# DonghuiZhuo/kube-batch-1

Measured on AMD Instinct MI355X. Metric: pod placements/sec + p50 session latency, 100k nodes × 1M pods, higher is better.
Workload: dtype int64

## Files before the change

kube-batch-1_amd/csrc/engine/engine_placer.h:

```cpp
#pragma once
#include <hip/hip_runtime.h>

#define KBHIP_STAMPS_OFF
#include "../kbhip_batch.h"
#include "../kbhip_engine.h"
#include "engine_dev.h"

namespace kbhip {

static_assert(sizeof(Row) == 4 * (kPkFlags - kPkRow), "the package carries a Row as 28 32-bit words");
static_assert(kEngDescClass + sizeof(TaskClass) / 4 <= kEngDescWords, "a descriptor carries its class");

template <typename ET>
__device__ __forceinline__ Row eng_row_after(const TaskClass& c, const PlaceDec<ET>& D, const Row& base) {
    const int cc = D.cc > 0 ? D.cc : 0;
    const int na = cc < D.ap_l ? cc : D.ap_l;
    return apply_commits(base, c, na, cc - na);
}
template <typename ET>
__device__ __forceinline__ void eng_fit_vals(const Conf& cf, const NodeCols& nc, const DevTables& t,
                                             const TaskClass& c, const PopArgs& a, const PlaceDec<ET>& D,
                                             const Row& base, const int32_t* fit_in, uint32_t fit_raw, uint64_t* g0,
                                             uint64_t* g1) {
    uint32_t fb_base = 0, fb_post = 0;
// ... 127 lines not shown

__device__ __forceinline__ void eng_host_out(const EngArgs& A, EngPlacerLds& L, uint32_t p, uint32_t slot) {
    const int lane = threadIdx.x & 63;
    while (__hip_atomic_load(&L.gran_seq, __ATOMIC_RELAXED, __HIP_MEMORY_SCOPE_WORKGROUP) != (int)p) {
        if (!__hip_atomic_load(&L.ok, __ATOMIC_RELAXED, __HIP_MEMORY_SCOPE_WORKGROUP)) return;
        __builtin_amdgcn_s_sleep(1);
    }
    PopOut* out = (PopOut*)((char*)A.out + (size_t)slot * sizeof(PopOut));
    const uint64_t g = L.gran[lane];
    if (lane < 2 && L.gfit[lane])
        __hip_atomic_store(&out->fit[lane], L.gfit[lane], __ATOMIC_RELAXED, __HIP_MEMORY_SCOPE_SYSTEM);
    if (g) __hip_atomic_store(&out->g[lane], g, __ATOMIC_RELAXED, __HIP_MEMORY_SCOPE_SYSTEM);
    ETL(A, p, 8);
}

__device__ __forceinline__ void eng_drop_stale(EngPlacerLds& L, const PopArgs& a, uint32_t q) {
    const int lane = threadIdx.x & 63;
    EngRowCache& rc = L.rc;
    const int r1 = (int)((q + 3) % 4);
    const int stage = kEngStage + kEngPkgN * (int)(q % 2);
    L.s64[lane] = 0;
    const uint32_t k0 = L.pkey[q % 2][lane], k1 = L.pkey[q % 2][64 + lane];
    auto kept = [&](uint32_t k) {
        if (!k) return false;
        const int sl = rc_find(&rc, key_node(k, a));
        return !(sl >= 64 * r1 && sl < 64 * r1 + 64);
    };
    const bool c0 = kept(k0), c1 = kept(k1);
    const uint64_t m0 = __ballot(c0), m1 = __ballot(c1);
    const int q0 = __builtin_amdgcn_mbcnt_hi((uint32_t)(m0 >> 32), __builtin_amdgcn_mbcnt_lo((uint32_t)m0, 0));
    const int q1 = __popcll(m0) +
                   __builtin_amdgcn_mbcnt_hi((uint32_t)(m1 >> 32), __builtin_amdgcn_mbcnt_lo((uint32_t)m1, 0));
    __builtin_amdgcn_s_waitcnt(0xc07f);
    __builtin_amdgcn_wave_barrier();
    if (c0) L.s64[q0] = k0;
    if (c1 && q1 < 64) L.s64[q1] = k1;
    if (c0) rc_insert(&rc, key_node(k0, a), stage + lane);
    if (c1 && q1 < 64) rc_insert(&rc, key_node(k1, a), stage + 64 + lane);
}

struct FrontKey {
    uint32_t e, fb, kind;
    int32_t na, s1p;
};
__device__ __forceinline__ FrontKey front_key(const Conf& cf, const NodeCols& nc, const DevTables& t,
                                              const TaskClass& c, const PopArgs& a, int node, const Row& r,
                                              uint8_t fl) {
    FrontKey k{0u, 0u, 0u, 0, INT32_MIN};
    const uint64_t pw[4] = {0, 0, 0, 0};
    int32_t sc;
    bool passed;
    const bool st = static_pred_f(cf, c, t, nc, node, fl);
    k.na = (st && cf.score_mult) ? na_weight(c, t, nc, node) : 0;
    const uint64_t k0 = dyn_key(cf, c, t, nc, r, pw, node, st, k.na, &sc, &passed);
    k.e = sweep_key<uint32_t>(k0, a);
    k.fb = fit_bits(c, r, passed);
    k.kind = k0 ? key_kind(k0) : 0;
    if (__ballot(k.kind == 2) != 0 && k.kind == 2) {
        const uint64_t k1 = dyn_key(cf, c, t, nc, apply_commits(r, c, 0, 1), pw, node, true, k.na, &sc, &passed);
        k.s1p = k1 ? key_score(k1) : INT32_MIN;
    }
    return k;
}
__device__ __forceinline__ int32_t front_s1a(const Conf& cf, const NodeCols& nc, const DevTables& t,
                                             const TaskClass& c, int node, const Row& r) {
    const uint64_t pw[4] = {0, 0, 0, 0};
    int32_t sc;
    bool passed;
    const int32_t na = cf.score_mult ? na_weight(c, t, nc, node) : 0;
    const uint64_t k1 = dyn_key(cf, c, t, nc, apply_commits(r, c, 1, 0), pw, node, true, na, &sc, &passed);
    return k1 ? key_score(k1) : INT32_MIN;
}
__device__ __forceinline__ bool front_wait(const EngPlacerLds& L, const int* seq, int want) {
    while (__hip_atomic_load(seq, __ATOMIC_RELAXED, __HIP_MEMORY_SCOPE_WORKGROUP) != want) {
        if (!__hip_atomic_load(&L.ok, __ATOMIC_RELAXED, __HIP_MEMORY_SCOPE_WORKGROUP)) return false;
        __builtin_amdgcn_s_sleep(1);
    }
    return true;
}

template <bool LIST>
__device__ __forceinline__ void eng_front_eval(const Conf& cf, const NodeCols& nc, const DevTables& t,
                                               const EngArgs& A, EngPlacerLds& L, uint32_t q, uint32_t dw, int set,
                                               int role) {
    const int lane = eng_lane();
    uint32_t w[8];
#pragma unroll
    for (int i = 0; i < 8; ++i) w[i] = (uint32_t)__builtin_amdgcn_readlane((int)dw, i);
    const EngDesc d = eng_decode(w);
    const PopArgs a = eng_args(d);
    const TaskClass c = eng_class_x(dw);
    const int ring = (int)((q + 3 - set) % 4);
    const int sl = 64 * ring + lane;
    if (!LIST && set == 0) {
        if (!front_wait(L, &L.rows_seq, (int)(q - 1))) return;
        const int node = L.xn[ring][lane];
        if (role == 0) {
            ETL(A, q - 1, 32);
            FrontKey k{0u, 0u, 0u, 0, INT32_MIN};
            if (node >= 0) k = front_key(cf, nc, t, c, a, node, L.rc.row[sl], L.flags[sl]);
            ETL(A, q - 1, 33);
            L.fe[0][lane] = k.e;
            L.ffb[0][lane] = (uint8_t)k.fb;
            L.fkind[0][lane] = (uint8_t)k.kind;
            L.fna[0][lane] = k.na;
            if (k.kind == 2) L.fs1p[0][lane] = k.s1p;
            ETL(A, q - 1, 34);
            L.e[0][lane] = wave_sort_desc(node >= 0 ? k.e : 0u);
            L.fbp[0][lane] = node >= 0 ? (uint8_t)k.fb : (uint8_t)0;
            __builtin_amdgcn_s_waitcnt(0xc07f);
            if (lane == 0) __hip_atomic_store(&L.sort_seq[0], (int)q, __ATOMIC_RELAXED, __HIP_MEMORY_SCOPE_WORKGROUP);
            ETL(A, q - 1, 35);
// ... 473 lines not shown
```

kube-batch-1_amd/csrc/kbhip_batch.h:

```cpp
#pragma once
#include <hip/hip_runtime.h>

#include "kbhip_eval.h"
#include "kbhip_internal.h"

namespace kbhip {

#if defined(KBHIP_STAMPS) && !defined(KBHIP_STAMPS_OFF)
static __device__ uint64_t* g_stamps;
#define STAMP(slot)                                                       \
    do {                                                                  \
        if (threadIdx.x == 0) g_stamps[(slot)] = __builtin_amdgcn_s_memrealtime(); \
    } while (0)
#else
#define STAMP(slot) do {} while (0)
#endif

#ifdef KBHIP_TIMELINE
constexpr int kTlSlots = 32768, kTlEvents = 32;
constexpr int kTlbSamples = 512, kTlbBlocks = 256;
static __constant__ uint64_t* g_tl;
#define TL(seq, ev)                                                                             \
    do {                                                                                        \
        if (g_tl) g_tl[((seq) % kTlSlots) * kTlEvents + (ev)] = __builtin_amdgcn_s_memrealtime(); \
// ... 717 lines not shown
        } else {
            const int32_t s0 = key_score(K), sm = key_score(Km);
            const int32_t rm = s1d < s0 ? s1d : s0;
            reach = rm > sm || (rm == sm && n < key_idx(Km));
        }
    }
    uint64_t alive = __ballot(reach);
    const int ap_own = K && key_kind(K) == 2 ? 0 : 64;
    if (Km && !alive && !every_member) {
        const bool inm = lane < m;
        const ET L = inm ? depth_entry<ET>(key_score(K), n, 0, a) : (ET)0;
        return tail(true, L, inm, lane, inm ? key_kind(K) : 0, ap_own);
    }
    q_cnt[lane] = 0;
    q_apos[lane] = ap_own;
    q_rm[lane] = K ? key_score(K) : 0;
    q_dl[lane] = 0;
    q_kind[0][lane] = K ? (uint8_t)key_kind(K) : (uint8_t)0;
    for (int h = lane; h < kHash; h += 64) q_hkey[h] = -1;
    __builtin_amdgcn_s_waitcnt(0xc07f);
    __builtin_amdgcn_wave_barrier();
    if (n >= 0) {
        int h = hash_slot(n);
        while (atomicCAS(&q_hkey[h], -1, n) != -1) h = (h + 1) & (kHash - 1);
        q_hlane[h] = lane;
    }
    ET L = K ? depth_entry<ET>(key_score(K), n, 0, a) : (ET)0;
    while (alive) {
        const int k = __popcll(alive);
        const int lk = k <= 1 ? 0 : k <= 2 ? 1 : k <= 4 ? 2 : k <= 8 ? 3 : k <= 16 ? 4 : k <= 32 ? 5 : 6;
        const int Dd = 64 >> lk;
        if ((alive >> lane) & 1)
            q_rl[__builtin_amdgcn_mbcnt_hi((uint32_t)(alive >> 32), __builtin_amdgcn_mbcnt_lo((uint32_t)alive, 0))] = lane;
        q_alive[lane] = 0;
        __builtin_amdgcn_s_waitcnt(0xc07f);
        __builtin_amdgcn_wave_barrier();
        const int seg = lane >> (6 - lk), off = lane & (Dd - 1);
        int j = seg < k ? q_rl[seg] : -1;
        const int dl = j >= 0 ? q_dl[j] : 0;
        const int d = dl + 1 + off;
        const int lastoff = (Dd < 63 - dl ? Dd : 63 - dl) - 1;
        if (off > lastoff) j = -1;
        Row bj{};
        int32_t naj = 0, rm0 = 0;
        int nj = -1, apj = 64;
        if (j >= 0) {
            const int sl = rc_slots[j];
            nj = key_idx(K0[j]);
            bj = rc->row[sl];
            naj = rc->na[sl];
            rm0 = q_rm[j];
            apj = q_apos[j];
        }
        auto eval_at = [&](int dd, int ap, int32_t* sc) -> int {
            const int na = dd < ap ? dd : ap;
            const Row r = apply_commits(bj, c, na, dd - na);
            int32_t s = 0;
            bool passed;
            const uint64_t kk = dyn_key(cf, c, t, nc, r, pw, nj, true, naj, &s, &passed);
            *sc = kk ? key_score(kk) : 0;
            return kk ? key_kind(kk) : 0;
        };
        int32_t sc = 0;
        int kd = j >= 0 ? eval_at(d, apj, &sc) : 0;
        int ap = (j >= 0 && kd == 2) ? d : 64;
        for (int o = 1; o < Dd; o <<= 1) {
            const int x = __shfl_xor(ap, o, 64);
            ap = x < ap ? x : ap;
        }
        ap = apj < ap ? apj : ap;
        const bool redo = j >= 0 && apj == 64 && d > ap;
        if (__ballot(redo) != 0 && redo) kd = eval_at(d, ap, &sc);
        bool ok = j >= 0 && kd != 0;
        int32_t rm = sc;
        for (int o = 1; o < Dd; o <<= 1) {
            const int32_t x = __shfl_up(rm, o, 64);
            const int y = __shfl_up((int)ok, o, 64);
            if (off >= o) {
                rm = x < rm ? x : rm;
                ok = ok && y;
            }
        }
        rm = rm0 < rm ? rm0 : rm;
        const ET e = ok ? depth_entry<ET>(rm, nj, d, a) : (ET)0;
        if (j >= 0) q_kind[d][j] = (uint8_t)kd;
        L = wave_merge_desc(L, wave_sort_desc(e));
        const ET T = readlane_t(L, m - 1);
        if (j >= 0 && off == lastoff) {
            q_rm[j] = rm;
            q_dl[j] = d;
            q_apos[j] = ap;
            q_alive[j] = (e != 0 && e >= T && d < 63) ? 1 : 0;
        }
        __builtin_amdgcn_s_waitcnt(0xc07f);
        __builtin_amdgcn_wave_barrier();
        alive = __ballot(q_alive[lane] != 0);
    }
    const bool inm = lane < m && L != 0;
    int lf = 0;
    if (inm) {
        const int ni = entry_node(L, a);
        int h = hash_slot(ni);
        while (q_hkey[h] != ni) h = (h + 1) & (kHash - 1);
        lf = q_hlane[h];
    }
    const int kind = inm ? q_kind[entry_depth(L)][lf] : 0;
    return tail(false, L, inm, lf, kind, q_apos[lane]);
}

template <typename ET>
__device__ __forceinline__ void place_fit_vals(const Conf& cf, const NodeCols& nc, const DevTables& t,
                                               const TaskClass& c, const PopArgs& a, const PlaceDec<ET>& D,
// ... 395 lines not shown
```

kube-batch-1_amd/csrc/kbhip_eval.h:

```cpp
#pragma once
#include <hip/hip_runtime.h>

#include <cmath>

#include "kbhip_internal.h"

#define KBHIP_HD __host__ __device__ __forceinline__

namespace kbhip {

struct Row {
    int64_t idle_cpu, idle_mem, idle_gpu, rel_cpu, rel_mem, rel_gpu, bf_cpu, bf_mem, bf_gpu;
    int64_t acpu, amem, nzc, nzm;
    int32_t pods, maxtasks;
};

struct ShardCand {
    uint64_t key;
    int32_t node;
    int32_t na;
    Row row;
    uint64_t pw[4];
};
struct ShardMsg {
// ... 52 lines not shown
        }
        case OP_EXISTS: return v >= 0;
        case OP_DNE: return v < 0;
        case OP_GT: return v >= 0 && t.valok[v] && t.valint[v] > r.rhs;
        case OP_LT: return v >= 0 && t.valok[v] && t.valint[v] < r.rhs;
    }
    return false;
}

KBHIP_HD bool term_match(const DevTables& t, const NodeCols& nc, const Term& tm, int n) {
    bool ok = true;
    for (int i = 0; i < tm.req_n; ++i) ok = ok && req_match(t, nc, t.reqs[tm.req_off + i], n);
    return ok;
}

KBHIP_HD bool static_pred_f(const Conf& cf, const TaskClass& c, const DevTables& t, const NodeCols& nc, int n,
                            uint8_t flags) {
    if (!cf.pred_on) return true;
    if (c.pred_err) return false;
    if (flags & 1) return false;
    for (int w = 0; w < nc.taint_words; ++w)
        if (nc.taints[(int64_t)w * nc.npad + n] & ~t.masks[c.tol_off + w]) return false;
    if (c.nsel_term >= 0 && !term_match(t, nc, t.terms[c.nsel_term], n)) return false;
    if (c.req_term_n >= 0) {
        bool any = false;
        for (int i = 0; i < c.req_term_n; ++i) any = any || term_match(t, nc, t.terms[c.req_term_off + i], n);
        if (!any) return false;
    }
    return true;
}
KBHIP_HD bool static_pred(const Conf& cf, const TaskClass& c, const DevTables& t, const NodeCols& nc, int n) {
    return static_pred_f(cf, c, t, nc, n, cf.pred_on ? nc.flags[n] : (uint8_t)0);
}

KBHIP_HD int32_t na_weight(const TaskClass& c, const DevTables& t, const NodeCols& nc, int n) {
    int32_t na = 0;
    for (int i = 0; i < c.pref_term_n; ++i) {
        const Term& tm = t.terms[c.pref_term_off + i];
        if (term_match(t, nc, tm, n)) na += tm.weight;
    }
    return na;
}

KBHIP_HD int64_t lr_score_f(int64_t req, int64_t cap, double f) {
    if (cap == 0 || req > cap) return 0;
    const int64_t num = (cap - req) * 10;
    int64_t q = (int64_t)(10.0 - 10.0 * f);
    q = q < 0 ? 0 : (q > 10 ? 10 : q);
    if (q * cap > num) --q;
    if ((q + 1) * cap <= num) ++q;
    return q;
}

KBHIP_HD int32_t node_score(const Conf& cf, const TaskClass& c, const Row& r, int32_t na, int32_t ipa) {
    if (!cf.score_mult) return 0;
    const int64_t rc = c.nz_cpu + r.nzc, rm = c.nz_mem + r.nzm;
    const double cpuF = r.acpu == 0 ? 1.0 : (double)rc / (double)r.acpu;
    const double memF = r.amem == 0 ? 1.0 : (double)rm / (double)r.amem;
    const int64_t lr = (lr_score_f(rc, r.acpu, cpuF) + lr_score_f(rm, r.amem, memF)) / 2;
    int64_t bra = 0;
    if (!(cpuF >= 1.0 || memF >= 1.0)) {
        const double d = fabs(cpuF - memF);
        const double one_minus = 1.0 - d;
        bra = (int64_t)(one_minus * 10.0);
    }
    return ((int32_t)lr * cf.w_lr + (int32_t)bra * cf.w_bra + na * cf.w_na + ipa * cf.w_pa) * cf.score_mult;
}

KBHIP_HD uint64_t dyn_key(const Conf& cf, const TaskClass& c, const DevTables& t,
                                            const NodeCols& nc, const Row& r, const uint64_t* portw,
                                            int n, bool stat_ok, int32_t na, int32_t* score_out, bool* passed,
                                            int32_t ipa = 0) {
    bool ok = stat_ok;
    if (cf.pred_on) {
        if (r.maxtasks <= r.pods) ok = false;
        if (c.has_ports)
            for (int w = 0; w < 4; ++w) if (w < port_win(c, nc))
                if (portw[w] & t.masks[c.pconf_off + w]) ok = false;
    }
    if (ok && c.score_err) ok = false;
    *passed = ok;
    if (!ok) return 0;
    const int32_t s = node_score(cf, c, r, na, ipa);
    *score_out = s;
    const bool fit_acc = c.ireq_cpu - (r.idle_cpu + r.bf_cpu) < kMinCPU &&
                         c.ireq_mem - (r.idle_mem + r.bf_mem) < kMinMem &&
                         c.ireq_gpu - (r.idle_gpu + r.bf_gpu) < kMinGPU;
    const bool fit_rel = c.ireq_cpu - r.rel_cpu < kMinCPU && c.ireq_mem - r.rel_mem < kMinMem &&
                         c.ireq_gpu - r.rel_gpu < kMinGPU;
    if (!fit_acc && !fit_rel) return 0;
    return pack_key(s, n + nc.base, fit_acc ? 0 : 1);
}

KBHIP_HD uint32_t fit_bits(const TaskClass& c, const Row& r, bool passed) {
    if (!passed) return 0;
    const int64_t ic = r.idle_cpu + r.bf_cpu, im = r.idle_mem + r.bf_mem, ig = r.idle_gpu + r.bf_gpu;
    const int64_t dc = c.req_cpu > 0 ? ic - (c.req_cpu + kMinCPU) : ic;
    const int64_t dm = c.req_mem > 0 ? im - (c.req_mem + kMinMem) : im;
    const int64_t dg = c.req_gpu > 0 ? ig - (c.req_gpu + kMinGPU) : ig;
    return 1u | (dc < 0 ? 2u : 0u) | (dm < 0 ? 4u : 0u) | (dg < 0 ? 8u : 0u);
}

KBHIP_HD uint64_t eval_node(const Conf& cf, const TaskClass& c, const DevTables& t,
                                              const NodeCols& nc, int n, int32_t* score_out, bool* passed,
                                              uint32_t* fit = nullptr) {
    const uint8_t fl = nc.flags[n];
    const Row r = load_row(nc, n);
    uint64_t pw[4] = {0, 0, 0, 0};
    if (c.has_ports)
        for (int w = 0; w < 4; ++w) if (w < port_win(c, nc)) pw[w] = nc.ports[port_at(c, nc, w, n)];
    const bool st = static_pred_f(cf, c, t, nc, n, fl);
    const int32_t na = (st && cf.score_mult) ? na_weight(c, t, nc, n) : 0;
    const uint64_t k = dyn_key(cf, c, t, nc, r, pw, n, st, na, score_out, passed);
    if (fit) *fit = fit_bits(c, r, *passed);
    return k;
}

KBHIP_HD uint64_t eval_node_walk(const Conf& cf, const TaskClass& c, const DevTables& t,
                                 const NodeCols& nc, int n, uint32_t* fit) {
    const Row r = load_row(nc, n);
    uint64_t pw[4] = {0, 0, 0, 0};
    if (c.has_ports)
        for (int w = 0; w < 4; ++w) if (w < port_win(c, nc)) pw[w] = nc.ports[port_at(c, nc, w, n)];
    const bool st = static_pred(cf, c, t, nc, n);
    const int32_t na = (st && cf.score_mult) ? na_weight(c, t, nc, n) : 0;
    int32_t s = 0;
    bool passed = false;
    uint64_t k = dyn_key(cf, c, t, nc, r, pw, n, st, na, &s, &passed);
    if (!k && passed && (r.bf_cpu | r.bf_mem | r.bf_gpu)) k = pack_key(s, n + nc.base, 0);
    *fit = fit_bits(c, r, passed);
    return k;
}

KBHIP_HD int32_t dom_g(const NodeCols& nc, int space, int g) {
    return nc.dom[(int64_t)space * nc.dom_stride + g];
}
// ... 128 lines not shown
```

kube-batch-1_amd/csrc/kbhip_types.h:

```cpp
#pragma once
#include <stdint.h>

namespace kbhip {

constexpr int kBlock = 256;
constexpr int kTopK = 64;
constexpr int kMaxChunk = 64;
constexpr int64_t kMinCPU = 10, kMinGPU = 10, kMinMem = 10LL * 1024 * 1024;

struct NodeCols {
    int64_t *idle_cpu, *idle_mem, *idle_gpu;
    int64_t *rel_cpu, *rel_mem, *rel_gpu;
    int64_t *bf_cpu, *bf_mem, *bf_gpu;
    int64_t *acpu, *amem;
    int64_t *nzc, *nzm;
    int32_t *pods, *maxtasks;
    uint8_t *flags;
    uint32_t *visits;
    int32_t *labels;
    uint64_t *taints;
    uint64_t *ports;
    int32_t *dom;
    int32_t n, npad, n_keys, taint_words, port_words;
    int32_t base;
    int32_t dom_stride;
};

enum : int32_t { OP_IN = 0, OP_NOTIN = 1, OP_EXISTS = 2, OP_DNE = 3, OP_GT = 4, OP_LT = 5,
                 OP_NAME_IN = 6, OP_NAME_NOTIN = 7, OP_FALSE = 8 };
struct Req {
    int32_t key;
    int32_t op;
    int32_t nvals;
    int32_t val_off;
    int64_t rhs;
};
struct Term {
    int32_t req_off, req_n;
    int32_t weight;
    int32_t pad;
};

struct TaskClass {
    int64_t ireq_cpu, ireq_mem, ireq_gpu;
    int64_t req_cpu, req_mem, req_gpu;
    int64_t nz_cpu, nz_mem;
    int32_t backfill;
    int32_t nsel_term;
    int32_t req_term_off, req_term_n;
    int32_t pref_term_off, pref_term_n;
    int32_t tol_off;
    int32_t pconf_off;
    int32_t pown_off;
    int32_t has_ports;
    int32_t pred_err;
    int32_t score_err;
    int32_t aff;
    int32_t ea_off, ea_n;
    int32_t pa_space, pa_cnt, pa_total, pa_self;
    int32_t paa_space, paa_cnt;
    int32_t ipa_off, ipa_n;
    int32_t upd_off, upd_n;
    int32_t pw_lo;
    int32_t dd_space;
    int32_t dd_ndom;
};
constexpr int kDedupMax = 1024;
constexpr int kPortWin = 4;

struct Conf {
    int32_t pred_on;
    int32_t score_mult;
    int32_t w_lr, w_bra, w_na, w_pa;
};

struct PopCtrl {
    int32_t stop;
    int32_t n_done;
    int32_t ready_count;
    int32_t min_avail;
    int32_t gang_mode;
    int32_t n_tasks;
    int32_t any_bf;
    int32_t fallback;
    int32_t mode;
    int32_t pad;
    uint32_t epoch;
    int32_t pad2;
    uint64_t* out;
    int32_t cls[kMaxChunk];
    int32_t res_node[kMaxChunk];
    int32_t res_kind[kMaxChunk];
    uint32_t arrive[kMaxChunk];
    uint64_t slot[kMaxChunk];
    int64_t ipa_lo[kMaxChunk];
    int64_t ipa_hi[kMaxChunk];
    int32_t fit[kMaxChunk][4];
};

struct CtrlInit {
    int32_t ready_count, min_avail, gang_mode, n_tasks, any_bf, fallback, mode;
    uint32_t epoch;
    uint64_t* out;
    int32_t cls[kMaxChunk];
};

__host__ __device__ inline uint64_t pack_key(int32_t score, int32_t idx, int32_t pipelined) {
    return ((uint64_t)((uint32_t)score ^ 0x80000000u) << 32) | ((uint64_t)(0x7fffffff - idx) << 1) |
           (uint64_t)(pipelined & 1);
}
__host__ __device__ inline int32_t key_idx(uint64_t k) { return 0x7fffffff - (int32_t)((k >> 1) & 0x7fffffff); }
__host__ __device__ inline int32_t key_score(uint64_t k) { return (int32_t)((uint32_t)(k >> 32) ^ 0x80000000u); }
__host__ __device__ inline int32_t key_kind(uint64_t k) { return (k & 1) ? 2 : 1; }

}
```

kube-batch-1_amd/csrc/session/02_open.cpp:

```cpp
#include "session.h"

namespace kbhip {

struct Encoder {
    const kbs::Snapshot& s;
    Session& S;
    Dict keys_all, vals, nss, taint_keys, port_keys, ip_dict, proto_dict;
    std::map<string, int> sel_keys;
    vector<Req> reqs;
    vector<Term> terms;
    vector<int32_t> vals_list;
    vector<uint64_t> masks;
    vector<int32_t> nl_off;
    vector<std::pair<int, int>> nl_kv;
    vector<std::tuple<string, string, string>> taint_defs;
    vector<std::tuple<int, int, int32_t>> port_defs;
    std::map<std::tuple<int, int, int32_t>, int> port_ids;
    int tw = 0, pw = 0;

    Encoder(const kbs::Snapshot& s_, Session& S_) : s(s_), S(S_) {}

    vector<int32_t> V32(const char* n) { return s.vec<int32_t>(n); }

    int sel_key(const string& k) {
// ... 926 lines not shown
            for (auto& id : v) id = new_id[id];
        E.port_ids.clear();
    }
    E.pw = ((int)E.port_defs.size() + 63) / 64;
    {
        int zero_ip = E.ip_dict.get("0.0.0.0");
        for (size_t ci = 0; ci < S.classes.size(); ++ci) {
            TaskClass& c = S.classes[ci];
            int lo = INT32_MAX, hi = -1;
            auto touch = [&](int id) { lo = std::min(lo, id); hi = std::max(hi, id); };
            for (int id : pod_ports[cls_pod[ci]]) {
                auto [ip, pr, port] = E.port_defs[id];
                touch(id);
                for (size_t u = 0; u < E.port_defs.size(); ++u) {
                    auto [uip, upr, uport] = E.port_defs[u];
                    if (upr != pr || uport != port) continue;
                    if (ip == zero_ip || uip == zero_ip || uip == ip) touch((int)u);
                }
            }
            c.pw_lo = hi < 0 ? 0 : lo / 64;
            if (hi >= 0 && hi / 64 - c.pw_lo >= kPortWin)
                fail_unsupported("a pod's host ports and their conflicts span more than " +
                                 std::to_string(kPortWin * 64) + " port ids");
            vector<uint64_t> conf(kPortWin, 0), own(kPortWin, 0);
            for (int id : pod_ports[cls_pod[ci]]) {
                auto [ip, pr, port] = E.port_defs[id];
                own[id / 64 - c.pw_lo] |= 1ULL << (id % 64);
                for (size_t u = 0; u < E.port_defs.size(); ++u) {
                    auto [uip, upr, uport] = E.port_defs[u];
                    if (upr != pr || uport != port) continue;
                    if (ip == zero_ip || uip == zero_ip || uip == ip) conf[u / 64 - c.pw_lo] |= 1ULL << (u % 64);
                }
            }
            c.pconf_off = (int32_t)E.masks.size();
            for (auto x : conf) E.masks.push_back(x);
            c.pown_off = (int32_t)E.masks.size();
            for (auto x : own) E.masks.push_back(x);
        }
    }
    S.n_spaces = aff.n_spaces;
    if (encode_only) {
        S.h_dom = aff.dom;
        S.h_aff_cnt = aff.cnt;
        S.h_aff_scalar = aff.scalar;
        S.h_aff_items = aff_items;
    } else {
        HIPCHK(hipSetDevice(device));
        S.device = device;
        S.stream = MemPool::get().take_stream();
        S.ov_streams[0] = S.stream;
        for (int k = 1; k <= kMaxDep; ++k) S.ov_streams[k] = MemPool::get().take_stream();
    }
    mark("classes");
    const int lo = (int)((int64_t)N * S.rank / S.world), hi = (int)((int64_t)N * (S.rank + 1) / S.world);
    const int nl = hi - lo, npl = std::max(((nl + kBlock - 1) / kBlock) * kBlock, kBlock);
    vector<int64_t> col[13];
    for (int i = 0; i < 13; ++i) col[i].assign(npl, 0);
    for (int i = lo; i < hi; ++i) {
        const int r = i - lo;
        col[0][r] = idle[i].c; col[1][r] = idle[i].m; col[2][r] = idle[i].g;
        col[3][r] = rel[i].c; col[4][r] = rel[i].m; col[5][r] = rel[i].g;
        col[6][r] = bf[i].c; col[7][r] = bf[i].m; col[8][r] = bf[i].g;
        col[9][r] = acpu[i]; col[10][r] = amem[i]; col[11][r] = nzc[i]; col[12][r] = nzm[i];
    }
    int64_t** dst[13] = {&S.nc.idle_cpu, &S.nc.idle_mem, &S.nc.idle_gpu, &S.nc.rel_cpu, &S.nc.rel_mem, &S.nc.rel_gpu,
                         &S.nc.bf_cpu, &S.nc.bf_mem, &S.nc.bf_gpu, &S.nc.acpu, &S.nc.amem, &S.nc.nzc, &S.nc.nzm};
    for (int i = 0; i < 13; ++i) *dst[i] = upload(S, S.b_cols[i], col[i]);
    vector<int32_t> pods_col(npl, 0), max_col(npl, 0);
    vector<uint8_t> flags_col(npl, 0);
    for (int i = lo; i < hi; ++i) {
        pods_col[i - lo] = podcnt[i];
        max_col[i - lo] = (int32_t)apods[i];
        flags_col[i - lo] = (!unsched.empty() && unsched[i]) ? 1 : 0;
    }
    S.nc.pods = upload(S, S.b_cols[13], pods_col);
    S.nc.maxtasks = upload(S, S.b_cols[14], max_col);
    S.nc.flags = upload(S, S.b_cols[15], flags_col);
    S.nc.visits = S.b_cols[16].alloc<uint32_t>(npl, encode_only);
    if (!encode_only) HIPCHK(hipMemsetAsync(S.nc.visits, 0, (size_t)npl * sizeof(uint32_t), S.stream));
    const int K = (int)E.sel_keys.size();
    vector<int32_t> lab((size_t)std::max(K, 1) * npl, -1);
    for (auto& kv : E.sel_keys) {
        auto kit = E.keys_all.ids.find(kv.first);
        if (kit == E.keys_all.ids.end()) continue;
        int kid = kit->second;
        for (int i = lo; i < hi; ++i)
            for (int q = E.nl_off[i]; q < E.nl_off[i + 1]; ++q)
                if (E.nl_kv[q].first == kid) lab[(size_t)kv.second * npl + (i - lo)] = E.nl_kv[q].second;
    }
    S.nc.labels = upload(S, S.b_labels, lab);
    vector<uint64_t> tcol((size_t)std::max(E.tw, 1) * npl, 0);
    for (int i = lo; i < hi; ++i)
        for (int id : node_taints[i]) tcol[(size_t)(id / 64) * npl + (i - lo)] |= 1ULL << (id % 64);
    S.nc.taints = upload(S, S.b_taints, tcol);
    vector<uint64_t> pcol((size_t)std::max(E.pw, 1) * npl, 0);
    for (int i = lo; i < hi; ++i)
        for (int id : node_ports[i]) pcol[(size_t)(id / 64) * npl + (i - lo)] |= 1ULL << (id % 64);
    S.nc.ports = upload(S, S.b_ports, pcol);
    S.n_aff_cnt = aff.active ? aff.cnt.size() : 1;
    S.n_aff_scalar = aff.active ? aff.scalar.size() : 1;
    if (aff.active) {
        S.nc.dom = upload(S, S.b_dom, aff.dom);
        if (aff_items.empty()) aff_items.push_back(0);
        S.tab.aff_items = upload(S, S.b_aff_items, aff_items);
        S.tab.aff_cnt = upload(S, S.b_aff_cnt, aff.cnt);
        S.tab.aff_scalar = upload(S, S.b_aff_scalar, aff.scalar);
// ... 119 lines not shown
```

kube-batch-1_amd/csrc/session/06_carry.cpp:

```cpp
#include "session.h"

namespace kbhip {

struct SavedOptions {
    bool batched, keys32, bf_batch, aff_batch, aff_fence, shard_overlap, rank_group, force_radix, debug_keys;
    int64_t time_every;
    int speculate, overlap, rank_first;
    bool engine, eng_quick, eng_lists, eng_timeline;
    int eng_nw_opt, eng_ng_opt;
};
static SavedOptions save_options(const Session& S) {
    return SavedOptions{S.batched, S.keys32, S.bf_batch, S.aff_batch, S.aff_fence, S.shard_overlap, S.rank_group,
                        S.force_radix,
                        S.debug_keys,
                        S.time_every, S.speculate, S.overlap, S.rank_first,
                        S.engine, S.eng_quick, S.eng_lists, S.d_eng_tl != nullptr,
                        S.eng_nw_opt, S.eng_ng_opt};
}
static void restore_options(Session& S, const SavedOptions& o) {
    S.batched = o.batched; S.keys32 = o.keys32; S.bf_batch = o.bf_batch; S.aff_batch = o.aff_batch;
    S.aff_fence = o.aff_fence;
    S.shard_overlap = o.shard_overlap;
    S.rank_group = o.rank_group; S.force_radix = o.force_radix; S.time_every = o.time_every;
    S.speculate = o.speculate; S.overlap = o.overlap; S.rank_first = o.rank_first;
// ... 556 lines not shown
        col[9][n] = acpu[n]; col[10][n] = amem[n];
        maxc[n] = (int32_t)apods[n];
        flg[n] = (!unsched.empty() && unsched[n]) ? 1 : 0;
    }
    {
        const int kThreads = host_threads();
        const int nth = P < (1 << 15) ? 1 : kThreads;
        vector<int> nb(nth + 1);
        for (int t = 0; t <= nth; ++t) nb[t] = (int)((int64_t)N * t / nth);
        vector<vector<vector<int32_t>>> bucket(nth, vector<vector<int32_t>>(nth));
        auto fill = [&](int t) {
            const int lo = (int)((int64_t)P * t / nth), hi = (int)((int64_t)P * (t + 1) / nth);
            for (int i = lo; i < hi; ++i) {
                const HPod& p = pods[i];
                if (!on_node_of(p)) continue;
                int r = (int)((int64_t)p.node * nth / N);
                while (r > 0 && p.node < nb[r]) --r;
                while (r + 1 < nth && p.node >= nb[r + 1]) ++r;
                bucket[t][r].push_back(i);
            }
        };
        {
            vector<std::thread> th;
            for (int t = 1; t < nth; ++t) th.emplace_back(fill, t);
            fill(0);
            for (auto& x : th) x.join();
        }
        auto rows = [&](int t) {
            for (int b = 0; b < nth; ++b)
            for (int i : bucket[b][t]) {
                const HPod& p = pods[i];
                const int n = p.node;
                if (p.backfill) { col[6][n] += p.req.c; col[7][n] += p.req.m; col[8][n] += p.req.g; }
                if (p.status == Releasing) { col[3][n] += p.req.c; col[4][n] += p.req.m; col[5][n] += p.req.g; }
                col[0][n] -= p.req.c; col[1][n] -= p.req.m; col[2][n] -= p.req.g;
                S.used[n].c += p.req.c; S.used[n].m += p.req.m; S.used[n].g += p.req.g;
                podcnt[n]++;
                col[11][n] += p.nzc;
                col[12][n] += p.nzm;
                for (int k = port_off[i]; k < port_off[i + 1]; ++k) {
                    const int id = port_ids[k];
                    pcol[(size_t)(id / 64) * S.nc.npad + n] |= 1ULL << (id % 64);
                }
            }
        };
        vector<std::thread> th;
        for (int t = 1; t < nth; ++t) th.emplace_back(rows, t);
        rows(0);
        for (auto& x : th) x.join();
    }
    S.any_bf = 0;
    for (int n = 0; n < N; ++n) if (col[6][n] || col[7][n] || col[8][n]) S.any_bf = 1;
    mark("rows");
    int64_t uploaded = 0;
    HIPCHK(hipStreamSynchronize(S.stream));
    size_t ci = 0;
    vector<RowPatch> patches;
    auto sync_col = [&](void* dptr, const void* want, size_t elem) {
        if (ci >= dcols.size() || dcols[ci].d != dptr || dcols[ci].elem != elem)
            throw Error(KBHIP_EDEVICE, "carry: device row read-back out of order");
        const uint8_t* hv = stage.p + dcols[ci++].off;
        const uint8_t* w = (const uint8_t*)want;
        auto scan = [&](auto zero) {
            using T = decltype(zero);
            const T* a = reinterpret_cast<const T*>(hv);
            const T* b = reinterpret_cast<const T*>(w);
            for (int n = 0; n < Nl; ++n) {
                if (a[n] == b[n]) continue;
                patches.push_back({(uint64_t)(uintptr_t)((T*)dptr + n), (uint64_t)b[n], (int32_t)sizeof(T), 0});
                uploaded += (int64_t)sizeof(T);
            }
        };
        if (elem == 8) scan(uint64_t{0});
        else if (elem == 4) scan(uint32_t{0});
        else scan(uint8_t{0});
    };
    for (int k = 0; k < 13; ++k) sync_col(dcol[k], col[k].data(), sizeof(int64_t));
    HIPCHK(hipMemsetAsync(S.nc.visits, 0, (size_t)S.nc.npad * sizeof(uint32_t), S.stream));
    S.fit_task = -1;
    sync_col(S.nc.pods, podcnt.data(), sizeof(int32_t));
    sync_col(S.nc.maxtasks, maxc.data(), sizeof(int32_t));
    sync_col(S.nc.flags, flg.data(), sizeof(uint8_t));
    for (int w = 0; w < S.nc.port_words; ++w)
        sync_col(S.nc.ports + (size_t)w * S.nc.npad, pcol.data() + (size_t)w * S.nc.npad, sizeof(uint64_t));
    DevBuf d_patch;
    if (!patches.empty()) {
        RowPatch* dp = d_patch.alloc<RowPatch>(patches.size());
        HIPCHK(hipMemcpyAsync(dp, patches.data(), patches.size() * sizeof(RowPatch), hipMemcpyHostToDevice, S.stream));
        HIPCHK(launch_row_patch(dp, (int)patches.size(), S.stream));
    }
    if (!new_classes.empty()) {
        S.class_kf.resize(S.classes.size());
        S.class_srange.resize(S.classes.size());
        static const vector<Term> no_terms;
        for (int ci : new_classes) class_key_format(S, S.classes[ci], no_terms, N, &S.class_kf[ci], &S.class_srange[ci]);
        S.tab.classes = upload(S, S.b_classes, S.classes);
        S.tab.masks = upload(S, S.b_masks, S.keep.masks);
        uploaded += (int64_t)(S.classes.size() * sizeof(TaskClass) + S.keep.masks.size() * sizeof(uint64_t));
    }
    HIPCHK(hipStreamSynchronize(S.stream));
    mark("upload");
    spare_pods().give(S.pods);
    S.pods.swap(pods);
    S.pod_port_off.swap(port_off);
    S.pod_port_ids.swap(port_ids);
    S.jobs.swap(jobs);
// ... 39 lines not shown
```

kube-batch-1_amd/csrc/session/07_abi.cpp:

```cpp
#include "session.h"

using namespace kbhip;

extern "C" {
int kbhip_session_carry(kb_session* s, int64_t* out_uploaded_bytes) {
    ABI_GUARD_S(s, {
        if (!s) throw kbhip::Error(KBHIP_EINVAL, "null session");
        if (s->s.encode_only) throw kbhip::Error(KBHIP_EINVAL, "encode-only session has no device state");
        kbhip::require_no_tickets(s->s);
        HIPCHK(hipSetDevice(s->s.device));
        session_carry(s->s);
        if (out_uploaded_bytes) *out_uploaded_bytes = s->s.carry_bytes;
        return 0;
    })
}
int kbhip_session_carry_events(kb_session* s, const int32_t* pods, const uint8_t* events, int64_t n,
                               int64_t* out_uploaded_bytes) {
    ABI_GUARD_S(s, {
        if (!s) throw kbhip::Error(KBHIP_EINVAL, "null session");
        if (n < 0 || (n > 0 && (!pods || !events))) throw kbhip::Error(KBHIP_EINVAL, "null argument");
        if (s->s.encode_only) throw kbhip::Error(KBHIP_EINVAL, "encode-only session has no device state");
        kbhip::require_no_tickets(s->s);
        HIPCHK(hipSetDevice(s->s.device));
        session_carry(s->s, pods, events, n);
// ... 394 lines not shown
                                       c.score_err, 0};
                v.insert(v.end(), f, f + 16);
            }
        } else if (n == "aff_dom") {
            if (!S.encode_only) throw kbhip::Error(KBHIP_EINVAL, "tables are kept by encode-only sessions");
            v = S.h_dom;
        } else if (n == "aff_cnt" || n == "aff_scalar") {
            if (S.encode_only) {
                v = n == "aff_cnt" ? S.h_aff_cnt : S.h_aff_scalar;
            } else {
                v.resize(n == "aff_cnt" ? S.n_aff_cnt : S.n_aff_scalar);
                HIPCHK(hipSetDevice(S.device));
                kbhip::ov_quiesce(s->s);
                HIPCHK(hipStreamSynchronize(S.stream));
                HIPCHK(hipMemcpy(v.data(), n == "aff_cnt" ? S.tab.aff_cnt : S.tab.aff_scalar, v.size() * 4,
                                 hipMemcpyDeviceToHost));
            }
        } else if (n == "aff_items") {
            v = S.h_aff_items;
        } else if (n == "dbg_keys") {
            const int64_t bytes = (int64_t)(S.dbg_keys.size() * 8);
            if (out && cap_bytes >= bytes && bytes) std::memcpy(out, S.dbg_keys.data(), (size_t)bytes);
            return bytes;
        } else if (n == "node_idle" || n == "node_backfilled" || n == "node_visits") {
            if (!S.encode_only) throw kbhip::Error(KBHIP_EINVAL, "node tables are read from encode-only sessions");
            const int64_t N = S.nc.n;
            if (n == "node_visits") {
                const int64_t bytes = N * (int64_t)sizeof(uint32_t);
                if (out && cap_bytes >= bytes && bytes) std::memcpy(out, S.nc.visits, (size_t)bytes);
                return bytes;
            }
            const bool idle = n == "node_idle";
            const int64_t* col[3] = {idle ? S.nc.idle_cpu : S.nc.bf_cpu, idle ? S.nc.idle_mem : S.nc.bf_mem,
                                     idle ? S.nc.idle_gpu : S.nc.bf_gpu};
            const int64_t bytes = N * 3 * (int64_t)sizeof(int64_t);
            if (out && cap_bytes >= bytes)
                for (int64_t i = 0; i < N; ++i)
                    for (int k = 0; k < 3; ++k) ((int64_t*)out)[3 * i + k] = col[k][i];
            return bytes;
        } else if (n == "dbg_pods") {
            v = S.dbg_pods;
        } else if (n == "engine_tl") {
            if (!S.d_eng_tl) throw kbhip::Error(KBHIP_EINVAL, "set option engine_timeline first");
            const int64_t bytes = (int64_t)kbhip::kEngTlSlots * kbhip::kEngTlEvents * 8;
            HIPCHK(hipSetDevice(S.device));
            kbhip::ov_quiesce(s->s);
            if (out && cap_bytes >= bytes) HIPCHK(hipMemcpy(out, S.d_eng_tl, (size_t)bytes, hipMemcpyDeviceToHost));
            return bytes;
        } else if (n == "pod_status" || n == "pod_node") {
            v.resize(S.pods.size());
            for (size_t i = 0; i < S.pods.size(); ++i) v[i] = n == "pod_status" ? S.pods[i].status : S.pods[i].node;
        } else if (n == "dims") {
            v = {S.nc.n, S.nc.npad, S.n_spaces, (int32_t)S.classes.size()};
        } else {
            throw kbhip::Error(KBHIP_EINVAL, "unknown table " + n);
        }
        const int64_t bytes = (int64_t)(v.size() * sizeof(int32_t));
        if (out && cap_bytes >= bytes && bytes) std::memcpy(out, v.data(), (size_t)bytes);
        return bytes;
    })
}
int kbhip_debug_replay(kb_session* s, int32_t n_steps, const int32_t* pods, const int32_t* modes,
                       const int32_t* nodes, const uint8_t* kinds, uint64_t* out_keys) {
    ABI_GUARD({
        if (!s || (n_steps && (!pods || !modes || !nodes || !kinds || !out_keys)))
            throw kbhip::Error(KBHIP_EINVAL, "null argument");
        kbhip::Session& S = s->s;
        if (!S.encode_only) throw kbhip::Error(KBHIP_EINVAL, "replay needs an encode-only session");
        using namespace kbhip;
        const NodeCols& nc = S.nc;
        const DevTables& t = S.tab;
        const int N = nc.n;
        int F = -1, any_bf = S.any_bf;
        vector<uint64_t> walk(N);
        for (int i = 0; i < n_steps; ++i) {
            if (pods[i] < 0 || pods[i] >= (int)S.pods.size() || S.pods[pods[i]].cls < 0)
                throw Error(KBHIP_EINVAL, "replay step is not a pending task");
            const TaskClass& c = S.classes[S.pods[pods[i]].cls];
            uint64_t* keys = out_keys + (int64_t)i * N;
            const bool first_fit = modes[i] == 1;
            const bool track = !first_fit && any_bf;
            int64_t lo = 0, hi = 0;
            if (!first_fit && c.ipa_n > 0)
                for (int n = 0; n < N; ++n) {
                    const int64_t v = ipa_count(c, t, nc, n, F);
                    lo = std::min(lo, v);
                    hi = std::max(hi, v);
                }
            for (int n = 0; n < N; ++n) {
                int32_t sc = 0;
                bool passed = false;
                keys[n] = first_fit ? eval_first_fit(S.conf, c, t, nc, n)
                                    : eval_node_aff(S.conf, c, t, nc, n, lo, hi, F, &sc, &passed);
                walk[n] = passed ? pack_key(sc, n + nc.base, 0) : 0;
            }
            const int w = nodes[i];
            if (w >= N) throw Error(KBHIP_EINVAL, "replay node out of range");
            const uint64_t k = w >= 0 ? keys[w] : 0;
            if (w >= 0 && !k) throw Error(KBHIP_EINVAL, "replay decision on a node with key 0");
            if (w >= 0) {
                const int kind = first_fit ? 1 : kinds[i];
                if (track) {
                    nc.idle_cpu[w] += nc.bf_cpu[w]; nc.idle_mem[w] += nc.bf_mem[w]; nc.idle_gpu[w] += nc.bf_gpu[w];
                    if (nc.bf_cpu[w] | nc.bf_mem[w] | nc.bf_gpu[w]) nc.visits[w] += 1;
                }
                commit_node(c, t, nc, w, kind);
// ... 46 lines not shown
```

kube-batch-1_amd/csrc/session/session.h:

```cpp
#pragma once
#include <hip/hip_runtime.h>
#include <rccl/rccl.h>

#include <algorithm>
#include <atomic>
#include <chrono>
#include <cmath>
#include <cstdio>
#include <cstdlib>
#include <cstring>
#include <deque>
#include <exception>
#include <map>
#include <memory>
#include <condition_variable>
#include <mutex>
#include <random>
#include <tuple>
#include <set>
#include <stdexcept>
#include <string>
#include <string_view>
#include <thread>
#include <unordered_map>
// ... 82 lines not shown
    static const int budget = [] {
        if (const char* e = std::getenv("KBHIP_HOST_THREADS")) {
            const int v = std::atoi(e);
            if (v >= 1 && v <= 64) return v;
        }
        const int hw = (int)std::thread::hardware_concurrency();
        return std::max(1, std::min(16, hw));
    }();
    return std::max(1, budget / std::max(1, g_live_sessions.load(std::memory_order_relaxed)));
}
inline int hw_queues() {
    const char* e = std::getenv("GPU_MAX_HW_QUEUES");
    const int v = e ? std::atoi(e) : 0;
    return v > 0 ? v : 4;
}
inline std::string mailbox_queue_check(int k, int queues) {
    const int per = 1 + kMaxDep;
    if (k <= 1 || k * per + 2 <= queues) return "";
    return "kbhip_shard_connect_mailbox: " + std::to_string(k) + " shard ranks of this process share one device; their " +
           std::to_string(k * per) + " streams exceed the process's " + std::to_string(queues) +
           " hardware queues (GPU_MAX_HW_QUEUES) with room for the runtime's own, so two ranks' mailbox kernels could "
           "wait on each other inside one queue: run one process per GPU, or set GPU_MAX_HW_QUEUES >= " +
           std::to_string(k * per + 2) +
           " before the process starts";
}
inline uint64_t process_token() {
    static const uint64_t tok = [] {
        std::random_device rd;
        uint64_t v = ((uint64_t)rd() << 32) ^ rd();
        v ^= (uint64_t)std::chrono::steady_clock::now().time_since_epoch().count() * 0x9e3779b97f4a7c15ull;
        return v ^ ((uint64_t)getpid() << 17);
    }();
    return tok;
}
struct HPod {
    int32_t uid_rank = 0;
    int ns = -1;
    int status = Pending;
    int32_t priority = 0;
    int64_t ts = 0;
    bool backfill = false;
    bool critical = false;
    bool node_rel = false;
    bool groupless = false;
    bool detached = false;
    R3 req, ireq;
    int64_t nzc = 0, nzm = 0;
    int job = -1;
    int cls = -1;
    int node = -1;
};
inline bool on_node_of(const HPod& p) {
    return p.node >= 0 && !p.detached && p.status != Succeeded && p.status != Failed;
}
inline int32_t dedup_space(const AffProgram& pg, const vector<int>& space_ndom) {
    if (pg.pa_space >= 0 || !pg.ipa.empty() || pg.pred_err) return -1;
    int32_t sp = pg.paa_space;
    vector<int32_t> offs;
    if (pg.paa_space >= 0) offs.push_back(pg.paa_cnt);
    for (size_t k = 0; k + 1 < pg.ea.size(); k += 2) {
        if (sp < 0) sp = pg.ea[k];
        if (pg.ea[k] != sp) return -1;
        offs.push_back(pg.ea[k + 1]);
    }
    if (sp < 0 || sp >= (int32_t)space_ndom.size() || space_ndom[sp] > kDedupMax) return -1;
    for (size_t k = 0; k + 2 < pg.upd.size(); k += 3)
        if (pg.upd[k] == UPD_CNT_ALLOC && pg.upd[k + 1] == sp &&
            std::find(offs.begin(), offs.end(), pg.upd[k + 2]) != offs.end())
            return sp;
    return -1;
}

struct HJob {
    int queue = -1;
    int32_t min_avail = 0, priority = 0;
    int32_t pg_priority = 0;
    bool shadow = false;
    int64_t ts = 0;
    vector<int> tasks;
    vector<int> pending;
    size_t cursor = 0;
    bool pending_built = false;
    bool maybe_pending = false;
    int cnt_alloc = 0, cnt_aob = 0;
    int32_t fit[4] = {0, 0, 0, 0};
    F3 drf_alloc;
    double drf_share = 0;
};
struct HQueue {
    string name;
    int32_t rank = 0;
    int32_t weight = 1;
    int64_t ts = 0;
    bool has_attr = false;
    F3 deserved, allocated, request;
    double share = 0;
};
struct CommPool {
    struct Entry {
        string id;
        int rank, world, device;
        ncclComm_t comm;
        bool busy;
    };
    std::mutex mu;
    vector<Entry> v;
// ... 850 lines not shown
```

Before: 3.081 million.

## Add range-checked fast path for node score using reciprocal division and 32-bit remainders

Adds a host-side check that all node allocatable and nonzero-request values stay below 2^52 across possible commits. When the check passes, node scoring converts int64 to double with a bit trick instead of a full conversion. It divides using a hardware reciprocal refined by Newton steps, computed once per row and reused across repeated evaluations, and uses 32-bit remainder arithmetic in the least-requested score. This targets the slow int64-to-double conversion and IEEE double-division sequences in the hot scoring loops. The cost is an O(pods+nodes) host scan at open and carry time, plus reliance on the refined reciprocal giving correctly rounded quotients.

```diff
diff --git a/kube-batch-1_amd/csrc/engine/engine_placer.h b/kube-batch-1_amd/csrc/engine/engine_placer.h
--- a/kube-batch-1_amd/csrc/engine/engine_placer.h
+++ b/kube-batch-1_amd/csrc/engine/engine_placer.h
@@ -203,12 +203,16 @@
     bool passed;
     const bool st = static_pred_f(cf, c, t, nc, node, fl);
     k.na = (st && cf.score_mult) ? na_weight(c, t, nc, node) : 0;
-    const uint64_t k0 = dyn_key(cf, c, t, nc, r, pw, node, st, k.na, &sc, &passed);
+    ScoreDen den{};
+    if (cf.inrange) den = score_den(r);
+    const ScoreDen* dp = cf.inrange ? &den : nullptr;
+    const uint64_t k0 = dyn_key(cf, c, t, nc, r, pw, node, st, k.na, &sc, &passed, 0, dp);
     k.e = sweep_key<uint32_t>(k0, a);
     k.fb = fit_bits(c, r, passed);
     k.kind = k0 ? key_kind(k0) : 0;
     if (__ballot(k.kind == 2) != 0 && k.kind == 2) {
-        const uint64_t k1 = dyn_key(cf, c, t, nc, apply_commits(r, c, 0, 1), pw, node, true, k.na, &sc, &passed);
+        const uint64_t k1 =
+            dyn_key(cf, c, t, nc, apply_commits(r, c, 0, 1), pw, node, true, k.na, &sc, &passed, 0, dp);
         k.s1p = k1 ? key_score(k1) : INT32_MIN;
     }
     return k;
diff --git a/kube-batch-1_amd/csrc/kbhip_batch.h b/kube-batch-1_amd/csrc/kbhip_batch.h
--- a/kube-batch-1_amd/csrc/kbhip_batch.h
+++ b/kube-batch-1_amd/csrc/kbhip_batch.h
@@ -793,12 +793,15 @@
             rm0 = q_rm[j];
             apj = q_apos[j];
         }
+        ScoreDen den{};
+        if (cf.inrange) den = score_den(bj);
+        const ScoreDen* dp = cf.inrange ? &den : nullptr;
         auto eval_at = [&](int dd, int ap, int32_t* sc) -> int {
             const int na = dd < ap ? dd : ap;
             const Row r = apply_commits(bj, c, na, dd - na);
             int32_t s = 0;
             bool passed;
-            const uint64_t kk = dyn_key(cf, c, t, nc, r, pw, nj, true, naj, &s, &passed);
+            const uint64_t kk = dyn_key(cf, c, t, nc, r, pw, nj, true, naj, &s, &passed, 0, dp);
             *sc = kk ? key_score(kk) : 0;
             return kk ? key_kind(kk) : 0;
         };
diff --git a/kube-batch-1_amd/csrc/kbhip_eval.h b/kube-batch-1_amd/csrc/kbhip_eval.h
--- a/kube-batch-1_amd/csrc/kbhip_eval.h
+++ b/kube-batch-1_amd/csrc/kbhip_eval.h
@@ -128,8 +128,74 @@
     return q;
 }
 
-KBHIP_HD int32_t node_score(const Conf& cf, const TaskClass& c, const Row& r, int32_t na, int32_t ipa) {
+KBHIP_HD double f64_inrange(int64_t v) {
+    return __builtin_bit_cast(double, (uint64_t)v | 0x4330000000000000ull) - 4503599627370496.0;
+}
+KBHIP_HD double rcp_inrange(double b) {
+#if defined(__HIP_DEVICE_COMPILE__)
+    const double x0 = __builtin_amdgcn_rcp(b);
+    const double x1 = __builtin_fma(x0, __builtin_fma(-b, x0, 1.0), x0);
+    return __builtin_fma(x1, __builtin_fma(-b, x1, 1.0), x1);
+#else
+    (void)b;
+    return 0.0;
+#endif
+}
+KBHIP_HD double div_den(double a, double b, double inv) {
+#if defined(__HIP_DEVICE_COMPILE__)
+    const double q = a * inv;
+    return __builtin_fma(__builtin_fma(-b, q, a), inv, q);
+#else
+    (void)inv;
+    return a / b;
+#endif
+}
+KBHIP_HD double div_inrange(double a, double b) { return div_den(a, b, rcp_inrange(b)); }
+
+struct ScoreDen {
+    double cap_c, inv_c, cap_m, inv_m;
+};
+KBHIP_HD ScoreDen score_den(const Row& r) {
+    ScoreDen d;
+    d.cap_c = f64_inrange(r.acpu);
+    d.cap_m = f64_inrange(r.amem);
+    d.inv_c = rcp_inrange(d.cap_c);
+    d.inv_m = rcp_inrange(d.cap_m);
+    return d;
+}
+
+KBHIP_HD int32_t lr_score_inrange(int64_t req, int64_t cap, double f) {
+    if (cap == 0 || req > cap) return 0;
+    int32_t q = (int32_t)(10.0 - 10.0 * f);
+    q = q < 0 ? 0 : (q > 10 ? 10 : q);
+    if (cap < ((int64_t)1 << 28)) {
+        const uint32_t cap32 = (uint32_t)cap;
+        const int32_t rem = (int32_t)((cap32 - (uint32_t)req) * 10u - (uint32_t)q * cap32);
+        return q + (rem >= (int32_t)cap32 ? 1 : 0) - (rem < 0 ? 1 : 0);
+    }
+    const int64_t rem = (cap - req) * 10 - (int64_t)q * cap;
+    return q + (rem >= cap ? 1 : 0) - (rem < 0 ? 1 : 0);
+}
+
+KBHIP_HD int32_t node_score_inrange(const Conf& cf, const TaskClass& c, const Row& r, const ScoreDen& den,
+                                    int32_t na, int32_t ipa) {
+    const int64_t rc = c.nz_cpu + r.nzc, rm = c.nz_mem + r.nzm;
+    const double cpuF = r.acpu == 0 ? 1.0 : div_den(f64_inrange(rc), den.cap_c, den.inv_c);
+    const double memF = r.amem == 0 ? 1.0 : div_den(f64_inrange(rm), den.cap_m, den.inv_m);
+    const int32_t lr = (lr_score_inrange(rc, r.acpu, cpuF) + lr_score_inrange(rm, r.amem, memF)) >> 1;
+    int32_t bra = 0;
+    if (!(cpuF >= 1.0 || memF >= 1.0)) {
+        const double d = fabs(cpuF - memF);
+        const double one_minus = 1.0 - d;
+        bra = (int32_t)(one_minus * 10.0);
+    }
+    return (lr * cf.w_lr + bra * cf.w_bra + na * cf.w_na + ipa * cf.w_pa) * cf.score_mult;
+}
+
+KBHIP_HD int32_t node_score(const Conf& cf, const TaskClass& c, const Row& r, int32_t na, int32_t ipa,
+                            const ScoreDen* den = nullptr) {
     if (!cf.score_mult) return 0;
+    if (cf.inrange) return node_score_inrange(cf, c, r, den ? *den : score_den(r), na, ipa);
     const int64_t rc = c.nz_cpu + r.nzc, rm = c.nz_mem + r.nzm;
     const double cpuF = r.acpu == 0 ? 1.0 : (double)rc / (double)r.acpu;
     const double memF = r.amem == 0 ? 1.0 : (double)rm / (double)r.amem;
@@ -146,7 +212,7 @@
 KBHIP_HD uint64_t dyn_key(const Conf& cf, const TaskClass& c, const DevTables& t,
                                             const NodeCols& nc, const Row& r, const uint64_t* portw,
                                             int n, bool stat_ok, int32_t na, int32_t* score_out, bool* passed,
-                                            int32_t ipa = 0) {
+                                            int32_t ipa = 0, const ScoreDen* den = nullptr) {
     bool ok = stat_ok;
     if (cf.pred_on) {
         if (r.maxtasks <= r.pods) ok = false;
@@ -157,7 +223,7 @@
     if (ok && c.score_err) ok = false;
     *passed = ok;
     if (!ok) return 0;
-    const int32_t s = node_score(cf, c, r, na, ipa);
+    const int32_t s = node_score(cf, c, r, na, ipa, den);
     *score_out = s;
     const bool fit_acc = c.ireq_cpu - (r.idle_cpu + r.bf_cpu) < kMinCPU &&
                          c.ireq_mem - (r.idle_mem + r.bf_mem) < kMinMem &&
diff --git a/kube-batch-1_amd/csrc/kbhip_types.h b/kube-batch-1_amd/csrc/kbhip_types.h
--- a/kube-batch-1_amd/csrc/kbhip_types.h
+++ b/kube-batch-1_amd/csrc/kbhip_types.h
@@ -72,6 +72,7 @@
     int32_t pred_on;
     int32_t score_mult;
     int32_t w_lr, w_bra, w_na, w_pa;
+    int32_t inrange;
 };
 
 struct PopCtrl {
diff --git a/kube-batch-1_amd/csrc/session/02_open.cpp b/kube-batch-1_amd/csrc/session/02_open.cpp
--- a/kube-batch-1_amd/csrc/session/02_open.cpp
+++ b/kube-batch-1_amd/csrc/session/02_open.cpp
@@ -1002,6 +1002,7 @@
         for (int k = 1; k <= kMaxDep; ++k) S.ov_streams[k] = MemPool::get().take_stream();
     }
     mark("classes");
+    S.conf.inrange = score_inrange(S.conf.pred_on != 0, S.pods, N, acpu.data(), amem.data(), nzc.data(), nzm.data(), apods.data());
     const int lo = (int)((int64_t)N * S.rank / S.world), hi = (int)((int64_t)N * (S.rank + 1) / S.world);
     const int nl = hi - lo, npl = std::max(((nl + kBlock - 1) / kBlock) * kBlock, kBlock);
     vector<int64_t> col[13];
diff --git a/kube-batch-1_amd/csrc/session/06_carry.cpp b/kube-batch-1_amd/csrc/session/06_carry.cpp
--- a/kube-batch-1_amd/csrc/session/06_carry.cpp
+++ b/kube-batch-1_amd/csrc/session/06_carry.cpp
@@ -632,6 +632,8 @@
     S.any_bf = 0;
     for (int n = 0; n < N; ++n) if (col[6][n] || col[7][n] || col[8][n]) S.any_bf = 1;
     mark("rows");
+    S.conf.inrange = score_inrange(S.conf.pred_on != 0, pods, N, col[9].data(), col[10].data(), col[11].data(),
+                                   col[12].data(), maxc.data());
     int64_t uploaded = 0;
     HIPCHK(hipStreamSynchronize(S.stream));
     size_t ci = 0;
diff --git a/kube-batch-1_amd/csrc/session/07_abi.cpp b/kube-batch-1_amd/csrc/session/07_abi.cpp
--- a/kube-batch-1_amd/csrc/session/07_abi.cpp
+++ b/kube-batch-1_amd/csrc/session/07_abi.cpp
@@ -470,6 +470,8 @@
             for (size_t i = 0; i < S.pods.size(); ++i) v[i] = n == "pod_status" ? S.pods[i].status : S.pods[i].node;
         } else if (n == "dims") {
             v = {S.nc.n, S.nc.npad, S.n_spaces, (int32_t)S.classes.size()};
+        } else if (n == "score_inrange") {
+            v = {S.conf.inrange};
         } else {
             throw kbhip::Error(KBHIP_EINVAL, "unknown table " + n);
         }
diff --git a/kube-batch-1_amd/csrc/session/session.h b/kube-batch-1_amd/csrc/session/session.h
--- a/kube-batch-1_amd/csrc/session/session.h
+++ b/kube-batch-1_amd/csrc/session/session.h
@@ -158,6 +158,27 @@
 };
 inline bool on_node_of(const HPod& p) {
     return p.node >= 0 && !p.detached && p.status != Succeeded && p.status != Failed;
+}
+template <typename MT>
+inline int32_t score_inrange(bool pred_on, const vector<HPod>& pods, int N, const int64_t* acpu, const int64_t* amem,
+                             const int64_t* nzc, const int64_t* nzm, const MT* maxtasks) {
+    constexpr int64_t kLim = (int64_t)1 << 52;
+    int64_t mc = 0, mm = 0, pending = 0;
+    for (const HPod& p : pods) {
+        if (p.nzc < 0 || p.nzm < 0 || p.nzc >= kLim || p.nzm >= kLim) return 0;
+        if (p.cls < 0 && p.status != Pending) continue;
+        mc = std::max(mc, p.nzc);
+        mm = std::max(mm, p.nzm);
+        ++pending;
+    }
+    for (int n = 0; n < N; ++n) {
+        if (acpu[n] < 0 || amem[n] < 0 || acpu[n] >= kLim || amem[n] >= kLim) return 0;
+        if (nzc[n] < 0 || nzm[n] < 0 || nzc[n] >= kLim || nzm[n] >= kLim) return 0;
+        const int64_t mt = std::max<int64_t>((int32_t)maxtasks[n], 0);
+        const int64_t cnt = (pred_on ? std::min(pending, mt) : pending) + 65;
+        if (mc > (kLim - 1 - nzc[n]) / cnt || mm > (kLim - 1 - nzm[n]) / cnt) return 0;
+    }
+    return 1;
 }
 inline int32_t dedup_space(const AffProgram& pg, const vector<int>& space_ndom) {
     if (pg.pa_space >= 0 || !pg.ipa.empty() || pg.pred_err) return -1;
```

New measurement: 3.039 million. -1.4%, worse.
